# yskft04/NGT

Measured on AMD Instinct MI355X. Metric: QPS at recall@10=0.95, 1M x 128-d float L2; achieved HBM GB/s vs peak, higher is better.
Workload: dtype f32

## Files before the change

### include/ngt_amd.h

```cpp
#ifndef NGT_AMD_H
#define NGT_AMD_H

#include <stddef.h>
#include <stdint.h>

#ifdef __cplusplus
extern "C" {
#endif

#define NGT_AMD_DISTANCE_L1 0
#define NGT_AMD_DISTANCE_L2 1
#define NGT_AMD_DISTANCE_HAMMING 2
#define NGT_AMD_DISTANCE_ANGLE 3
#define NGT_AMD_DISTANCE_COSINE 4
#define NGT_AMD_DISTANCE_NORMALIZED_ANGLE 5
#define NGT_AMD_DISTANCE_NORMALIZED_COSINE 6
#define NGT_AMD_DISTANCE_JACCARD 7
#define NGT_AMD_DISTANCE_SPARSE_JACCARD 8
#define NGT_AMD_DISTANCE_NORMALIZED_L2 9
#define NGT_AMD_DISTANCE_POINCARE 100
#define NGT_AMD_DISTANCE_LORENTZ 101
#define NGT_AMD_OBJECT_UINT8 1
#define NGT_AMD_OBJECT_FLOAT 2

// ... 60 lines not shown

int ngt_amd_linear_search(ngt_amd_index *index, const void *queries, uint32_t nq, uint32_t k,
                          double radius, uint32_t *ids, float *dists, uint32_t *n);
int ngt_amd_linear_search_device(ngt_amd_index *index, const void *d_queries,
                                 uint64_t query_bytes, uint32_t nq, uint32_t k, double radius,
                                 uint32_t *d_ids, float *d_dists, uint32_t *d_n, void *stream);

int ngt_amd_distances(ngt_amd_index *index, const void *queries, uint32_t nq,
                      const uint32_t *qidx, const uint32_t *oid, uint64_t npairs, float *out);

int ngt_amd_prepare_queries_device(ngt_amd_index *index, const float *d_in, uint32_t nq,
                                   void *d_out, void *stream);

float ngt_amd_last_search_kernel_ms(const ngt_amd_index *index);
int ngt_amd_last_search_filtered(const ngt_amd_index *index);
int ngt_amd_stream_error_word(ngt_amd_index *index, void *stream, int *word);
uint32_t ngt_amd_last_search_slots(const ngt_amd_index *index);
uint32_t ngt_amd_last_search_budget(const ngt_amd_index *index);

#define NGT_AMD_GRAPH_ANNG 1
#define NGT_AMD_GRAPH_KNNG 2
#define NGT_AMD_GRAPH_ONNG 4
#define NGT_AMD_GRAPH_IANNG 5
typedef struct {
  int32_t edge_size_for_creation;
  int32_t edge_size_for_search;
  int32_t batch_size_for_creation;
  int32_t seed_size;
  float epsilon_for_creation;
  int32_t graph_type;
// ... 192 lines not shown
int ngt_amd_ngtq_open(const char *path, int device, ngt_amd_index **out);
int ngt_amd_ngtq_set(ngt_amd_index *index, const float *local, uint32_t N, uint32_t dsub,
                     const uint64_t *list_off, uint64_t nlists, const uint32_t *eids,
                     const uint16_t *elids, uint64_t nentries, const float *objects,
                     uint64_t object_records);
int ngt_amd_ngtq_search(ngt_amd_index *index, const ngt_amd_ngtq_search_params *params,
                        const float *queries, uint32_t nq, uint32_t *ids, float *dists, uint32_t *n);
int ngt_amd_ngtq_search_device(ngt_amd_index *index, const ngt_amd_ngtq_search_params *params,
                               const void *d_queries, uint64_t query_bytes, uint32_t nq,
                               uint32_t *d_ids, float *d_dists, uint32_t *d_n, void *stream);

int ngt_amd_test_unchecked_set(int device, int tagged, int trim, const uint64_t *script,
                               const uint8_t *tag_lane, uint32_t n, uint32_t tail_cap,
                               uint32_t spill_cap, float expr, uint64_t *popped, uint32_t *npopped,
                               uint64_t *events, uint32_t *nevents, uint32_t *maxq, uint32_t *error);

#ifdef __cplusplus
}
#endif
#endif
```

### ngt_amd/_sigs.py

```python
from ctypes import (POINTER, Structure, c_bool, c_char_p, c_double, c_float, c_int, c_int16, c_int32,
                    c_int64, c_size_t, c_uint, c_uint8, c_uint32, c_uint64, c_void_p)


class SearchParams(Structure):
    _fields_ = [("k", c_uint32), ("epsilon", c_float), ("radius", c_float), ("edge_size", c_int64),
                ("seed_mode", c_int32), ("all_leaf_nodes", c_int32),
                ("visited_hash_log2", c_int32), ("distance_filter", c_int32)]


class QgSearchParams(Structure):
    _fields_ = [("k", c_uint32), ("epsilon", c_float), ("result_expansion", c_float), ("radius", c_float),
                ("seed_mode", c_int32), ("visited_hash_log2", c_int32)]


class NgtqSearchParams(Structure):
    _fields_ = [("size", c_uint32), ("expansion", c_float), ("epsilon", c_float), ("mode", c_int32)]


class BuildParams(Structure):
    _fields_ = [("edge_size_for_creation", c_int32), ("edge_size_for_search", c_int32),
                ("batch_size_for_creation", c_int32), ("seed_size", c_int32), ("epsilon_for_creation", c_float),
                ("graph_type", c_int32)]


# ... 87 lines not shown
        "ngt_amd_last_search_lookahead": (c_int, [vp]),
        "ngt_amd_qg_train_local_ngt": (c_int, [vp, c_uint64, c_uint32, c_uint32, vp]),
        "ngt_amd_search_device": (c_int, [vp, POINTER(SearchParams), vp, c_uint64, c_uint32, vp, vp, vp, vp,
                                          vp, vp, vp]),
        "ngt_amd_linear_search": (c_int, [vp, vp, c_uint32, c_uint32, c_double, vp, vp, vp]),
        "ngt_amd_linear_search_device": (c_int, [vp, vp, c_uint64, c_uint32, c_uint32, c_double, vp, vp, vp,
                                                 vp]),
        "ngt_amd_distances": (c_int, [vp, vp, c_uint32, vp, vp, c_uint64, vp]),
        "ngt_amd_prepare_queries_device": (c_int, [vp, vp, c_uint32, vp, vp]),
        "ngt_amd_srand": (None, [c_uint]),
        "ngt_amd_last_search_kernel_ms": (c_float, [vp]),
        "ngt_amd_last_search_slots": (c_uint32, [vp]),
        "ngt_amd_stream_error_word": (c_int, [vp, vp, vp]),
        "ngt_amd_last_search_budget": (c_uint32, [vp]),
        "ngt_amd_last_search_filtered": (c_int, [vp]),
        "ngt_amd_build_begin": (c_int, [vp, POINTER(BuildParams)]),
        "ngt_amd_build_set_onng_edges": (c_int, [vp, c_int32, c_int32]),
        "ngt_amd_build_insert": (c_int, [vp, c_uint64, c_uint64]),
        "ngt_amd_build_graph_size": (c_int, [vp, u64p, u64p]),
        "ngt_amd_build_get_graph": (c_int, [vp, vp, vp, vp]),
        "ngt_amd_build_tree_size": (c_int, [vp, u32p, u32p, u64p]),
        "ngt_amd_build_get_tree": (c_int, [vp, vp, vp, vp, vp, vp, vp, vp, vp, vp, vp]),
        "ngt_amd_build_set_graph": (c_int, [vp, vp, vp, vp, c_uint64]),
        "ngt_amd_build_set_tree": (c_int, [vp, vp, vp, vp, vp, vp, vp, c_uint32, vp, vp, vp, vp, c_uint32,
                                           c_uint32]),
        "ngt_amd_build_remove": (c_int, [vp, vp, c_uint64, vp]),
        "ngt_amd_build_longest_removed_list": (c_uint64, [vp]),
        "ngt_amd_remove_relink": (c_int, [vp, vp, c_uint32, vp, vp, vp]),
        "ngt_amd_remove_fast_path_capacity": (c_uint32, []),
        "ngt_amd_onng_reconstruct": (c_int, [c_int, vp, vp, vp, c_uint64, POINTER(OnngParams), u64p]),
# ... 35 lines not shown
        "ngt_amd_qg_code_stride": (c_uint64, [vp]),
        "ngt_amd_qg_record_bytes": (c_uint64, [vp]),
        "ngt_amd_qg_get_graph": (c_int, [vp, vp, vp]),
        "ngt_amd_qg_lut": (c_int, [vp, vp, c_uint32, vp, vp, vp]),
        "ngt_amd_qg_adc": (c_int, [vp, vp, vp, vp, c_uint32, vp, vp, c_uint64, vp, vp]),
        "ngt_amd_qg_search": (c_int, [vp, POINTER(QgSearchParams), vp, c_uint32, vp, vp, vp, vp, vp, vp]),
        "ngt_amd_qg_search_device": (c_int, [vp, POINTER(QgSearchParams), vp, c_uint64, c_uint32, vp, vp, vp,
                                             vp, vp, vp, vp]),
        "ngt_amd_ngtq_open": (c_int, [c_char_p, c_int, POINTER(vp)]),
        "ngt_amd_ngtq_set": (c_int, [vp, vp, c_uint32, c_uint32, vp, c_uint64, vp, vp, c_uint64, vp, c_uint64]),
        "ngt_amd_ngtq_search": (c_int, [vp, POINTER(NgtqSearchParams), vp, c_uint32, vp, vp, vp]),
        "ngt_amd_ngtq_search_device": (c_int, [vp, POINTER(NgtqSearchParams), vp, c_uint64, c_uint32, vp, vp, vp,
                                               vp]),
        "ngt_amd_test_unchecked_set": (c_int, [c_int, c_int, c_int, vp, vp, c_uint32, c_uint32, c_uint32, c_float,
                                               vp, vp, vp, vp, vp, vp]),
        "ngt_open_index": (vp, [c_char_p, vp]),
        "ngt_create_graph_and_tree": (vp, [c_char_p, vp, vp]),
        "ngt_create_graph_and_tree_in_memory": (vp, [vp, vp]),
        "ngt_create_property": (vp, [vp]),
        "ngt_save_index": (c_bool, [vp, c_char_p, vp]),
        "ngt_get_property": (c_bool, [vp, vp, vp]),
        "ngt_get_property_dimension": (c_int32, [vp, vp]),
        "ngt_set_property_dimension": (c_bool, [vp, c_int32, vp]),
        "ngt_set_property_edge_size_for_creation": (c_bool, [vp, c_int16, vp]),
        "ngt_set_property_edge_size_for_search": (c_bool, [vp, c_int16, vp]),
        "ngt_get_property_object_type": (c_int32, [vp, vp]),
        "ngt_is_property_object_type_float": (c_bool, [c_int32]),
        "ngt_is_property_object_type_integer": (c_bool, [c_int32]),
        "ngt_set_property_object_type_float": (c_bool, [vp, vp]),
        "ngt_set_property_object_type_integer": (c_bool, [vp, vp]),
# ... 90 lines not shown
```

### ngt_amd/csrc/index_internal.h

```cpp
#pragma once
#include <hip/hip_runtime.h>
#include <stdint.h>

#include <algorithm>
#include <atomic>
#include <mutex>
#include <string>
#include <vector>

#include "../../include/ngt_amd.h"
#include "ngt_kernels.h"
#include "search_plan.h"

namespace ngt_amd {

int fail(const char* fmt, ...);

#define HIP_OK(expr)                                                                     \
  do {                                                                                   \
    hipError_t e_ = (expr);                                                              \
    if (e_ != hipSuccess)                                                                \
      return ngt_amd::fail("%s failed: %s (%s:%d)", #expr, hipGetErrorString(e_), __FILE__, __LINE__); \
  } while (0)

// ... 94 lines not shown
  DevBuf<float> local;
  DevBuf<uint64_t> list_off;
  DevBuf<uint32_t> eids;
  DevBuf<uint16_t> elids;
  DevBuf<uint8_t> orows;
};

struct SearchCtx {
  hipStream_t stream = nullptr;
  DevBuf<uint32_t> work, seeds, seed_count, slot_epoch;
  DevBuf<uint64_t> seed_off, spill;
  DevBuf<uint8_t> vis;
  uint32_t slots = 0;
  uint32_t launch_slots = 0;
  bool launch_filtered = false;
  int launch_la = -1;
  uint64_t vis_stride = 0;
  hipEvent_t ev0 = nullptr, ev1 = nullptr;
  DevBuf<uint8_t> lut;
  DevBuf<float> scale, toff;
  DevBuf<uint64_t> partial;
  DevBuf<uint16_t> sqh, sql;
  DevBuf<float> shb;
  DevBuf<uint64_t> gthr;
  DevBuf<uint32_t> ivf_cid, ivf_cn;
  DevBuf<float> ivf_cd;
  DevBuf<int> err;
  DevBuf<uint8_t> qstate;
  DevBuf<uint32_t> qflag, order;
  DevBuf<float> prio;
// ... 93 lines not shown
  uint64_t nrows = 0;
  DevBuf<uint8_t> rows, valid;
  uint64_t rows_version = 0;
  struct {
    DevBuf<uint16_t> rh, rl;
    DevBuf<uint32_t> xmax;
    uint64_t version = ~0ull;
    int passes = 0;
  } scan;
  struct {
    DevBuf<uint8_t> codes;
    DevBuf<uint32_t> st;
    DevBuf<float> params;
    uint64_t stride = 0;
    uint64_t version = ~0ull;
  } filt;
  std::vector<uint8_t> h_valid;
  std::vector<uint64_t> h_degree_nonzero;
  DevBuf<uint64_t> edge_off;
  DevBuf<uint32_t> edges;
  uint64_t nedges = 0;
  DevBuf<uint32_t> adj;
  uint64_t adj_stride = 0;
  uint64_t max_degree = 0;
  uint64_t adj_version = 0;

  bool has_graph = false;
  std::vector<uint8_t> h_graph_empty;
  bool has_tree = false;
  bool tree_has_empty_leaf = false;
// ... 81 lines not shown
```

### ngt_amd/csrc/ngt_amd_api.cpp

```cpp
#include <hip/hip_runtime.h>
#include <math.h>
#include <stdarg.h>
#include <stdio.h>
#include <stdlib.h>
#include <string.h>

#include <algorithm>
#include <climits>
#include <cmath>
#include <cfloat>
#include <string>
#include <vector>

#include "../../include/ngt_amd.h"
#include "device_graph.h"
#include "index_internal.h"
#include "ngt_kernels.h"
#include "prep_kernels.h"

using namespace ngt_amd;

static thread_local std::string g_err;

int ngt_amd::fail(const char* fmt, ...) {
// ... 372 lines not shown
  t.seed_stride = stride;
  t.seed_count = c->seed_count.p;
  HIP_OK(launch_tree_seeds(t, ix->metric, ix->otype, s));
  return 0;
}

static int ensure_filter(ngt_amd_index* ix) {
  std::lock_guard<std::mutex> lk(ix->mu);
  if (ix->filt.version == ix->rows_version) return 0;
  ix->filt.stride = ix->dp <= 128 ? ix->dp : (ix->dp + 127) / 128 * 128;
  HIP_OK(ix->filt.codes.alloc((size_t)ix->nrows * ix->filt.stride));
  HIP_OK(ix->filt.st.alloc(8));
  HIP_OK(ix->filt.params.alloc(8));
  HIP_OK(launch_filter_build(ix->rows.p, ix->row_bytes, ix->nrows, ix->dp, ix->filt.stride, ix->filt.codes.p, ix->filt.st.p,
                             ix->filt.params.p, ix->stream));
  HIP_OK(hipStreamSynchronize(ix->stream));
  ix->filt.version = ix->rows_version;
  return 0;
}

int ngt_amd::fill_index_args(ngt_amd_index* ix, uint64_t es, SearchArgs& a) {
  a.rows = ix->rows.p;
  a.row_bytes = ix->row_bytes;
  a.nrows = (uint32_t)ix->nrows;
  a.dp = (int)ix->dp;
  a.edge_off = ix->edge_off.p;
  a.edges = ix->edges.p;
  a.edge_size = es;
  std::lock_guard<std::mutex> lk(ix->mu);
  const uint64_t need = adjacency_need(ix, es);
  if (build_padded_adjacency(ix, need)) return -1;
// ... 146 lines not shown
  a.la_sh_log2 = plan.la_sh_log2;
  a.lat_slots = plan.lat_slots;
  a.lat_tail = plan.lat_tail;
  a.lat_hop = plan.lat_hop;
  a.lat_feed = plan.lat_feed;
  a.out_ids = d_ids;
  a.out_dists = d_dists;
  a.out_n = d_n;
  a.counters = d_counters;
  a.error = c->err.p;
  if (plan.use_filter) {
    if (ensure_filter(ix)) return -1;
    a.fcodes = ix->filt.codes.p;
    a.fstride = ix->filt.stride;
    a.fparams = ix->filt.params.p;
  }
  c->launch_filtered = plan.use_filter;

  if (prm->seed_mode == NGT_AMD_SEED_TREE) {
    if (run_tree_seeds(ix, c, d_queries, query_bytes, nq, prm->k, prm->all_leaf_nodes, s)) return -1;
    if (ix->tree_has_empty_leaf && !ix->h_graph_empty.empty() && fill_empty_tree_seeds(ix, c, nq, s)) return -1;
    a.seeds = c->seeds.p;
    a.seed_stride = kTreeSeedStride;
    a.seed_count = c->seed_count.p;
  } else {
    if (!d_seeds || !d_seed_off) return fail("search: seed lists required for this seed mode");
    a.seeds = d_seeds;
    a.seed_off = d_seed_off;
  }
  if (!plan.error.empty()) return fail("%s", plan.error.c_str());
  if (ensure_vis_scratch(ix, c, plan.lds_bytes, nq, s)) return -1;
  a.vis = c->vis.p;
  a.vis_stride = c->vis_stride;
  a.slot_epoch = c->slot_epoch.p;
  a.spill = c->spill.p;
  a.spill_cap = ix->spill_cap;
  a.work = c->work.p;
  HIP_OK(hipMemsetAsync(c->work.p, 0, 3 * sizeof(uint32_t), s));
  const uint32_t slots = std::min<uint32_t>(c->slots, nq);
  c->launch_slots = slots;
  c->launch_la = plan.la_mode();
  return launch_planned(ix, c, plan, a, slots, s);
}

static std::mutex g_rand_mu;
static GlibcRandHost& seed_rand() {
  static GlibcRandHost r = [] {
    GlibcRandHost g;
    g.seed(1);
    return g;
  }();
  return r;
}

extern "C" void ngt_amd_srand(unsigned int seed) {
// ... 97 lines not shown
  hipStream_t s = (hipStream_t)stream;
  SearchCtx* c = ctx_for(ix, s);
  if (!c) return -1;
  if (run_tree_seeds(ix, c, d_queries, query_bytes, nq, k, 0, s)) return -1;
  HIP_OK(hipMemcpy2DAsync(d_seeds, (size_t)seed_stride * sizeof(uint32_t), c->seeds.p,
                          (size_t)kTreeSeedStride * sizeof(uint32_t), (size_t)kTreeSeedStride * sizeof(uint32_t), nq,
                          hipMemcpyDeviceToDevice, s));
  HIP_OK(hipMemcpyAsync(d_count, c->seed_count.p, (size_t)nq * sizeof(uint32_t), hipMemcpyDeviceToDevice, s));
  return 0;
}

extern "C" int ngt_amd_last_search_filtered(const ngt_amd_index* ix) {
  if (!ix) return 0;
  SearchCtx* c = ix->last_ctx.load();
  return c && c->launch_filtered ? 1 : 0;
}

extern "C" int ngt_amd_last_search_lookahead(const ngt_amd_index* ix) {
  if (!ix) return -1;
  SearchCtx* c = ix->last_ctx.load();
  return c ? c->launch_la : -1;
}

extern "C" uint32_t ngt_amd_last_search_budget(const ngt_amd_index* ix) {
  if (!ix) return 0;
  SearchCtx* c = ix->last_ctx.load();
  return c ? c->launch_budget : 0;
}

extern "C" int ngt_amd_stream_error_word(ngt_amd_index* ix, void* stream, int* word) {
// ... 466 lines not shown
```

### ngt_amd/csrc/ngt_kernels.h

```cpp
#pragma once
#include <hip/hip_runtime.h>
#include <stddef.h>
#include <stdint.h>
#include <stdlib.h>

#include <algorithm>

#include "knobs.h"

namespace ngt_amd {

struct DistanceArgs {
  const uint8_t* rows;
  uint64_t row_bytes;
  const uint8_t* queries;
  uint64_t query_bytes;
  const uint32_t* qidx;
  const uint32_t* oid;
  float* out;
  uint64_t npairs;
  int dp;
};

struct TreeSeedArgs {
// ... 39 lines not shown
  const uint32_t* seeds;
  const uint64_t* seed_off;
  uint32_t seed_stride;
  const uint32_t* seed_count;
  uint32_t k;
  float coef;
  float radius;
  uint64_t edge_size;
  uint32_t ht_log2;
  uint32_t cq_cap;
  uint32_t vf_log2;
  uint32_t accepted_only;
  const uint8_t* fcodes;
  uint64_t fstride;
  const float* fparams;
  uint32_t* out_ids;
  float* out_dists;
  uint32_t* out_n;
  uint64_t* counters;
  uint32_t* work;
  uint8_t* vis;
  uint64_t vis_stride;
  uint32_t* slot_epoch;
  uint64_t* spill;
  uint32_t spill_cap;
  int* error;
  uint32_t la_lmax;
  uint32_t la_sh_log2;
  uint32_t lat_slots;
  uint32_t lat_tail;
// ... 407 lines not shown
```

### ngt_amd/csrc/search_common.h

```cpp
#pragma once
#include <hip/hip_runtime.h>
#include <stdint.h>

#include "ngt_device.h"

namespace ngt_amd {

#ifdef NGT_AMD_STAMPS
__device__ __forceinline__ uint64_t stamp() {
  uint64_t t;
  __builtin_amdgcn_sched_barrier(0);
  asm volatile("s_memtime %0\n\ts_waitcnt lgkmcnt(0)" : "=s"(t)::"memory");
  __builtin_amdgcn_sched_barrier(0);
  return t;
}
#define NGT_MARK(dst)              \
  do {                             \
    const uint64_t now_ = stamp(); \
    dst += now_ - t_last;          \
    t_last = now_;                 \
  } while (0)
#else
#define NGT_MARK(dst)
#endif
// ... 354 lines not shown
#pragma unroll
    for (int j = 0; j < 4; j++) {
      if (j == 0 || r0 + 16 * j < m) {
        uint32_t qc = 0u, cc = 0u;
#pragma unroll
        for (int w = 0; w < NW; w++) {
          qc = __builtin_amdgcn_udot4(q[w].x, c[j][w].x, qc, false);
          qc = __builtin_amdgcn_udot4(q[w].y, c[j][w].y, qc, false);
          cc = __builtin_amdgcn_udot4(c[j][w].x, c[j][w].x, cc, false);
          cc = __builtin_amdgcn_udot4(c[j][w].y, c[j][w].y, cc, false);
        }
        const uint32_t s = quad_sum_u32(cc - 2u * qc);
        const int r = r0 + 16 * j + rs;
        if (g == 0 && r < m) out[r] = sq + s;
      }
    }
  }
}

__device__ __forceinline__ void filter_query(const float* qf, int dp, float fa, float fb, uint8_t* qb, uint32_t& sq,
                                             double& rq) {
  uint32_t s = 0u;
  double r2 = 0.0;
  for (int i = lane_id(); i < dp; i += 64) {
    float c = rintf((qf[i] - fa) / fb);
    c = c >= 0.0f ? (c <= 255.0f ? c : 255.0f) : 0.0f;
    qb[i] = (uint8_t)c;
    s += (uint32_t)c * (uint32_t)c;
    double t = ((double)qf[i] - (double)fa) / (double)fb;
    t = t < 0.0 ? 0.0 : (t > 255.0 ? 255.0 : t);
// ... 124 lines not shown
```

### ngt_amd/csrc/search_kernels.hip

```cpp
#include <hip/hip_runtime.h>
#include <stdint.h>
#include <stdlib.h>

#include "ngt_device.h"
#include "ngt_kernels.h"
#include "search_common.h"
#include "search_layout.h"

namespace ngt_amd {



template <int M, typename T>
__global__ void __launch_bounds__(256) ngt_distances_kernel(DistanceArgs a) {
  const int lane = threadIdx.x & 63;
  const int g = lane & 3;
  const uint64_t quad = ((uint64_t)blockIdx.x * blockDim.x + threadIdx.x) >> 2;
  const uint64_t nquads = ((uint64_t)gridDim.x * blockDim.x) >> 2;
  for (uint64_t i = quad; i < a.npairs; i += nquads) {
    const T* q = reinterpret_cast<const T*>(a.queries + (uint64_t)a.qidx[i] * a.query_bytes);
    const T* x = row_ptr<T>(a.rows, a.row_bytes, a.oid[i]);
    const float d = quad_distance<M, T>(q, x, a.dp, g);
    if (g == 0) a.out[i] = d;
  }
// ... 128 lines not shown
    const uint64_t key = rsp[i];
    spill[i] = key;
    remark(key_id(key));
  }
  for (uint32_t i = lane; i < hv.npop; i += 64) remark(rpop[i]);
  __syncthreads();
}

#ifndef NGT_AMD_C2_WPE
#define NGT_AMD_C2_WPE 4
#endif
template <int M, int NCH, int G>
constexpr int search_waves_per_simd() {
  return (NCH > 0 && G == 1) ? NGT_AMD_C2_WPE : (NCH < 0 ? (M == kL2 ? 4 : 3) : 2);
}
template <int M, typename T, int NCH, int G>
__global__ void __launch_bounds__(64, (search_waves_per_simd<M, NCH, G>())) ngt_graph_search_kernel(SearchArgs a) {
  extern __shared__ __attribute__((aligned(16))) uint8_t smem[];
  const int lane = lane_id();
  SearchState st;
  uint8_t* p = smem;
  const bool use_hash = a.ht_log2 != 0;
  st.ht = reinterpret_cast<uint32_t*>(p);
  if (use_hash) p += (size_t)4 << a.ht_log2;
  st.vf = a.vf_log2 ? reinterpret_cast<uint32_t*>(p) : nullptr;
  st.vf_shift = 32 - a.vf_log2;
  const uint32_t vf_words = a.vf_log2 ? (1u << a.vf_log2) / 32 : 0u;
  p += (size_t)4 * vf_words;
  st.cq = reinterpret_cast<uint64_t*>(p);
  p += (size_t)8 * a.cq_cap;
  uint64_t* cmin = reinterpret_cast<uint64_t*>(p);
  p += ((size_t)8 * ((a.cq_cap + 63) / 64) + 15) & ~(size_t)15;
  st.res = reinterpret_cast<uint64_t*>(p);
  p += ((size_t)8 * (a.k + 1) + 15) & ~(size_t)15;
  st.nid = reinterpret_cast<uint32_t*>(p);
  p += 256;
  st.nd = reinterpret_cast<float*>(p);
  p += 256;
  T* qlds = reinterpret_cast<T*>(p);
  p += ((size_t)a.dp * sizeof(T) + 15) & ~(size_t)15;
  constexpr bool kFilterable = NCH > 0 && (NCH & 1) == 0 && M == kL2 && sizeof(T) == 4;
  constexpr bool kFilterCos = NCH < 0 && (M == kCosine || M == kAngle) && sizeof(T) == 4;
  uint8_t* qb = p;
  uint32_t* surv = reinterpret_cast<uint32_t*>(p + (size_t)a.dp);
  bool use_filter = false;
  float fa = 0.f, fb = 0.f, fe = 0.f, fx = 0.f;
  if constexpr (kFilterable || kFilterCos) {
    if (a.fcodes != nullptr && a.fparams[4] != 0.0f) {
      use_filter = true;
      fa = a.fparams[0];
      fb = a.fparams[1];
      fe = a.fparams[2];
      fx = a.fparams[3];
      use_filter = fb > 0.0f;
    }
  }
  (void)qb; (void)surv; (void)fa; (void)fb; (void)fe; (void)fx;

  const uint32_t slot = blockIdx.x;
  uint8_t* vis = a.vis + (uint64_t)slot * a.vis_stride;
  uint64_t* spill = a.spill + (uint64_t)slot * a.spill_cap;
  const uint32_t hcap = use_hash ? 1u << a.ht_log2 : 0u;
  const uint32_t hlimit = hcap - (hcap >> 2);

  const uint32_t nwork = a.nwork_dev ? *a.nwork_dev : a.nq;
  for (;;) {
    uint32_t w = 0;
    if (lane == 0) w = atomicAdd(a.work, 1u);
    w = (uint32_t)__builtin_amdgcn_readfirstlane((int)w);
// ... 23 lines not shown
        filter_query(reinterpret_cast<const float*>(qlds), a.dp, fa, fb, qb, fsq, frq);
        finv_b = 1.0 / (double)fb;
        __syncthreads();
      }
    }
    CosFilterQuery fcq{};
    (void)fcq;
    if constexpr (kFilterCos) {
      if (use_filter) {
        filter_query_cos(reinterpret_cast<const float*>(qlds), a.dp, fa, fb, qb, fcq);
        __syncthreads();
      }
    }

    bool bitmap_mode = !use_hash;
    const bool lazy = a.accepted_only && !use_hash && st.vf;
    uint32_t nvisited = 0;
    uint32_t ncq = 0, nspill = 0, nres = 0, maxq = 0;
    uint64_t ndist = 0, nvisit = 0, nexp = 0, nedge = 0, nexact = 0;
    uint64_t t_pop = 0, t_adj = 0, t_filt = 0, t_eval = 0, t_last = 0, t_rest = 0;
    (void)t_pop; (void)t_adj; (void)t_filt; (void)t_eval; (void)t_last; (void)t_rest;
#ifdef NGT_AMD_STAMPS
    t_last = stamp();
#endif
    float radius = a.radius;
    const uint32_t k = a.k;

    const uint64_t sb = a.seed_off ? a.seed_off[qi] : (uint64_t)qi * a.seed_stride;
    const uint32_t ns = a.seed_off ? (uint32_t)(a.seed_off[qi + 1] - sb) : a.seed_count[qi];
    if (resume) {
      PauseHdr h;
// ... 8 lines not shown
      nexp = h.nexp;
      nedge = h.nedge;
      nexact = h.nexact;
      for (uint32_t c = 0; c < ((ncq + 63) >> 6); c++) cq_chunk_min(st.cq, cmin, ncq, c);
      __syncthreads();
    }
    for (uint32_t base = 0; base < (resume ? 0u : ns); base += 64) {
      const uint32_t m = ns - base < 64 ? ns - base : 64;
      if ((uint32_t)lane < m) st.nid[lane] = a.seeds[sb + base + lane];
      __syncthreads();
      eval_any<M, T, NCH, G>(qlds, a, qfold, st.nid, st.nd, (int)m);
      __syncthreads();
      if ((uint32_t)lane < m) {
        const uint32_t id = st.nid[lane];
        const uint64_t key = make_key(st.nd[lane], id);
        visit(a.ht_log2, st, id, bitmap_mode, vis, epoch);
        if (ncq + lane < a.cq_cap) st.cq[ncq + lane] = key;
        else spill[nspill + (ncq + lane - a.cq_cap)] = key;
      }
      __syncthreads();
      for (uint32_t j = 0; j < m; j++) {
        const float d = st.nd[j];
        if (d <= a.radius) res_insert(st.res, nres, k, make_key(d, st.nid[j]));
      }
      const uint32_t ncq0 = ncq;
      if (ncq + m <= a.cq_cap) {
        ncq += m;
      } else {
        nspill += ncq + m - a.cq_cap;
        ncq = a.cq_cap;
      }
      for (uint32_t c = ncq0 >> 6; c < ((ncq + 63) >> 6); c++) cq_chunk_min(st.cq, cmin, ncq, c);
      ndist += m;
      nvisited += m;
      __syncthreads();
      if (!bitmap_mode && nvisited > hlimit) {
        ht_to_vis(a.ht_log2, st, vis, epoch);
        bitmap_mode = true;
        __syncthreads();
      }
    }
    if (nres >= k) radius = key_dist(st.res[k - 1]);
    float expr = __fmul_rn(a.coef, radius);

    auto accept_batch = [&](const uint32_t* ids, uint32_t me) {
      uint64_t okmask = ballot64((uint32_t)lane < me && st.nd[lane] <= expr);
      while (okmask) {
        const int j = __ffsll((long long)okmask) - 1;
        okmask &= okmask - 1;
        const float d = st.nd[j];
        if (!(d <= expr)) continue;
        const uint64_t key = make_key(d, ids[j]);
        if (lazy && lane == 0) mark_accepted(st, ids[j], vis, epoch);
        if (ncq >= a.cq_cap) {
          ncq = compact(st.cq, ncq, expr);
          if (nspill) nspill = compact(spill, nspill, expr);
          for (uint32_t c = 0; c < ((ncq + 63) >> 6); c++) cq_chunk_min(st.cq, cmin, ncq, c);
          __builtin_amdgcn_wave_barrier();
// ... 7 lines not shown
          ncq++;
        } else {
          if (nspill >= a.spill_cap) {
            if (lane == 0) atomicOr(a.error, 1);
          } else {
            if (lane == 0) spill[nspill] = key;
            nspill++;
          }
        }
        if (ncq + nspill > maxq) maxq = ncq + nspill;
        if (d <= radius) {
          res_insert(st.res, nres, k, key);
          if (nres >= k) {
            radius = key_dist(st.res[k - 1]);
            expr = __fmul_rn(a.coef, radius);
          }
        }
        __builtin_amdgcn_wave_barrier();
      }
      __syncthreads();
      if (!bitmap_mode && nvisited > hlimit) {
        ht_to_vis(a.ht_log2, st, vis, epoch);
        bitmap_mode = true;
        __syncthreads();
      }
    };

    uint32_t pf_node = 0, pf0 = 0, pf1 = 0, pf2 = 0, pf3 = 0;
    (void)pf_node; (void)pf0; (void)pf1; (void)pf2; (void)pf3;

// ... 42 lines not shown
      } else {
        ncq--;
        __syncthreads();
        cq_chunk_min(st.cq, cmin, ncq, bidx >> 6);
        if ((ncq >> 6) != (bidx >> 6)) cq_chunk_min(st.cq, cmin, ncq, ncq >> 6);
        __syncthreads();
      }
      nexp++;
      NGT_MARK(t_pop);

      const uint32_t target = key_id(wbest);
      if (a.pause_after && lane == 0 && nexp <= a.pause_after + kPauseStepMax)
        reinterpret_cast<uint32_t*>(a.qstate + (uint64_t)qi * a.qstate_stride +
                                    PauseLayout(a.k, a.cq_cap, 0).off_pop)[nexp - 1] = target;
      uint64_t eb, deg;
      const bool padded = a.adj != nullptr;
      if (padded) {
        eb = (uint64_t)target * a.adj_stride;
        deg = a.adj_stride < a.edge_size ? a.adj_stride : a.edge_size;
      } else {
        eb = a.edge_off[target];
        deg = a.edge_off[target + 1] - eb;
        if (deg > a.edge_size) deg = a.edge_size;
      }

      if constexpr (kFilterable) {
        if (use_filter && lazy && padded && deg <= 256) {
          const uint32_t nchk = (uint32_t)((deg + 63) >> 6);
          uint32_t a0, a1, a2, a3;
          if (pf_node == target) {
            a0 = pf0; a1 = pf1; a2 = pf2; a3 = pf3;
          } else {
            load_adj_row(a.adj + eb, deg, a0, a1, a2, a3);
          }
          {
            uint64_t nb = ~0ull;
            const uint32_t nc2 = (ncq + 63) >> 6;
            if ((uint32_t)lane < nc2) nb = cmin[lane];
            if ((uint32_t)lane + 64 < nc2) { const uint64_t v = cmin[lane + 64]; nb = v < nb ? v : nb; }
            for (uint32_t i = lane; i < nspill; i += 64) { const uint64_t v = spill[i]; nb = v < nb ? v : nb; }
            nb = wave_min_u64(nb);
            pf_node = (nb != ~0ull && key_dist(nb) <= expr) ? key_id(nb) : 0u;
// ... 4 lines not shown
          for (uint32_t c = 0; c < nchk; c++) {
            const uint32_t id = c == 0 ? a0 : (c == 1 ? a1 : (c == 2 ? a2 : a3));
            const uint64_t vmask = ballot64(id != 0u);
            const uint32_t cnt = (uint32_t)__popcll(vmask);
            nedge += cnt;
            if (cnt == 0) break;
            bool bit = false;
            uint32_t pw = 0;
            if (id != 0u) {
              const uint32_t b = (id * 0x85EBCA77u) >> st.vf_shift;
              bit = ((st.vf[b >> 5] >> (b & 31)) & 1u) != 0u;
              if (bit)
                pw = __hip_atomic_load(reinterpret_cast<const uint32_t*>(vis + (id & ~3u)), __ATOMIC_RELAXED,
                                       __HIP_MEMORY_SCOPE_AGENT);
            }
            st.nid[lane] = id;
            __syncthreads();
            filter_l2u8<NCH>(qb, fsq, a.fcodes, st.nid, reinterpret_cast<uint32_t*>(st.nd), (int)cnt);
            __syncthreads();
            const bool fresh = id != 0u && (!bit || ((pw >> (8 * (id & 3))) & 0xffu) != epoch);
            const uint32_t m = (uint32_t)__popcll(ballot64(fresh));
            ndist += m;
            nvisit += m;
            nvisited += m;
            const uint32_t fthr = filter_threshold(expr, (double)fe, finv_b, frq);
            const bool keep = fresh && reinterpret_cast<const uint32_t*>(st.nd)[lane] <= fthr;
            const uint64_t km = ballot64(keep);
            const uint32_t me = (uint32_t)__popcll(km);
            nexact += me;
            NGT_MARK(t_filt);
            if (ns + me > 64) {
              eval_any<M, T, NCH, G>(qlds, a, qfold, surv, st.nd, (int)ns);
              __syncthreads();
              NGT_MARK(t_eval);
              accept_batch(surv, ns);
              ns = 0;
            }
            if (keep) surv[ns + mbcnt(km)] = id;
            ns += me;
            __syncthreads();
// ... 365 lines not shown
}

hipError_t launch_schedule(const uint32_t* qflag, const float* prio, uint32_t nq, uint32_t* order, uint32_t* n_out,
                           hipStream_t s) {
  hipLaunchKernelGGL(ngt_schedule_kernel, dim3(1), dim3(1024), 0, s, qflag, prio, nq, order, n_out);
  return hipGetLastError();
}

hipError_t launch_graph_search(const SearchArgs& a, int metric, int otype, uint32_t slots,
                               hipStream_t s) {
  if (a.nq == 0) return hipSuccess;
  const size_t lds = search_lds_bytes(a, otype);
  if (metric == kL2 && otype == kFloat && (a.dp == 128 || a.dp == 96)) {
    if (a.dp == 128 && slots < 512)
      hipLaunchKernelGGL((ngt_graph_search_kernel<kL2, float, 8, 4>), dim3(slots), dim3(64), lds, s, a);
    else if (a.dp == 128)
      hipLaunchKernelGGL((ngt_graph_search_kernel<kL2, float, 8, 1>), dim3(slots), dim3(64), lds, s, a);
    else
      hipLaunchKernelGGL((ngt_graph_search_kernel<kL2, float, 6, 1>), dim3(slots), dim3(64), lds, s, a);
    return hipGetLastError();
  }
  if (otype == kFloat && a.dp > 128 && ((a.dp >> 4) & 3) == 0 && !ngt_amd::knob("NGT_AMD_NO_STREAM")) {
    if (metric == kL2) {
      hipLaunchKernelGGL((ngt_graph_search_kernel<kL2, float, -1, 1>), dim3(slots), dim3(64), lds, s, a);
      return hipGetLastError();
    }
    if (metric == kCosine) {
      hipLaunchKernelGGL((ngt_graph_search_kernel<kCosine, float, -1, 1>), dim3(slots), dim3(64), lds, s, a);
      return hipGetLastError();
    }
    if (metric == kAngle) {
      hipLaunchKernelGGL((ngt_graph_search_kernel<kAngle, float, -1, 1>), dim3(slots), dim3(64), lds, s, a);
// ... 61 lines not shown
```

### ngt_amd/csrc/search_plan.cpp

```cpp
#include "search_plan.h"

#include <stdio.h>
#include <stdlib.h>

#include <algorithm>

#include "knobs.h"
#include "search_layout.h"

namespace ngt_amd {

PlanKnobs read_plan_knobs() {
  PlanKnobs kn;
  kn.la = knob("NGT_AMD_LA");
  kn.filter = knob("NGT_AMD_FILTER");
  kn.no_stream = knob("NGT_AMD_NO_STREAM");
  kn.adj = knob("NGT_AMD_ADJ");
  kn.ht_log2 = knob("NGT_AMD_HT_LOG2");
  kn.cq_cap = knob("NGT_AMD_CQ_CAP");
  kn.accepted_only = knob("NGT_AMD_ACCEPTED_ONLY");
  kn.vfilter = knob("NGT_AMD_VFILTER");
  kn.la_lmax = knob("NGT_AMD_LA_LMAX");
  kn.lat = knob("NGT_AMD_LAT");
  kn.lat_tail = knob("NGT_AMD_LAT_TAIL");
  kn.lat_slots = knob("NGT_AMD_LAT_SLOTS");
  kn.lat_hop = knob("NGT_AMD_LAT_HOP");
  kn.lat_feed = knob("NGT_AMD_LAT_FEED");
  kn.sched = knob("NGT_AMD_SCHED");
  kn.sched_frac = knob("NGT_AMD_SCHED_FRAC");
  kn.sched_b = knob("NGT_AMD_SCHED_B");
  return kn;
}

void apply_visited_knobs(const PlanKnobs& kn, uint32_t& ht_log2, uint32_t& cq_cap, uint32_t& vf_log2,
                         bool keep_filter) {
  if (const char* v = kn.ht_log2) ht_log2 = (uint32_t)std::max(8, std::min(15, atoi(v)));
  if (const char* v = kn.cq_cap) cq_cap = (uint32_t)std::max(64, std::min(8192, atoi(v)));
  if (const char* v = kn.vfilter) {
    const int f = atoi(v);
    if (f > 0) vf_log2 = (uint32_t)std::max(11, std::min(18, f));
    else if (!keep_filter) vf_log2 = 0u;
  }
}

namespace {
// ... 141 lines not shown
  if (la_mode == 1 && !(kn.lat && atoi(kn.lat) == 0) && list_cap(sh) <= 256u && k <= 64u)
    lat = plan_speculating(sh, k, kn, p);
  if (!lat && la_mode >= 0 && la_lds(sh, k, p, la_mode) > lds_max) la_mode = -1;
  if (!lat) {
    p.kernel = la_mode < 0 ? kPlanOneExpansion : la_mode == 0 ? kPlanLookaheadWave : kPlanLookaheadEight;
    p.lds_bytes = la_mode >= 0 ? la_lds(sh, k, p, la_mode) : one_lds(sh, k, p);
  }
  p.la_full = la_mode >= 0 && !lat && !p.accepted_only;
  if (p.lds_bytes > lds_max) {
    char buf[160];
    snprintf(buf, sizeof buf, "search: k=%u needs %zu bytes of LDS per query (max %zu)", k, p.lds_bytes, lds_max);
    p.error = buf;
  }
  p.sched_shape = p.kernel == kPlanOneExpansion && p.accepted_only && p.ht_log2 == 0 && p.vf_log2 != 0 && p.use_adj &&
                  p.use_filter && k <= 64;
  p.sched_on = p.sched_shape && (kn.sched ? atoi(kn.sched) : 1) != 0;
  p.sched_frac = kn.sched_frac ? std::max(0.01, std::min(0.9, atof(kn.sched_frac))) : 0.25;
  p.sched_forced = kn.sched_b ? (uint32_t)std::max(0, atoi(kn.sched_b)) : 0u;
  return p;
}

}
```

### ngt_amd/csrc/search_plan.h

```cpp
#pragma once
#include <stddef.h>
#include <stdint.h>

#include <string>

#include "../../include/ngt_amd.h"

namespace ngt_amd {

struct PlanShape {
  int metric, otype;
  uint32_t dp;
  uint64_t row_bytes, nrows;
  int cu_count;
  size_t lds_per_block, lds_per_cu;
  uint64_t adj_stride;
  uint64_t edge_size;
};

struct PlanKnobs {
  const char *la, *filter, *no_stream, *adj, *ht_log2, *cq_cap, *accepted_only, *vfilter, *la_lmax, *lat, *lat_tail,
      *lat_slots, *lat_hop, *lat_feed, *sched, *sched_frac, *sched_b;
};
PlanKnobs read_plan_knobs();

enum PlanKernel : int {
  kPlanOneExpansion = 0,
  kPlanLookaheadWave,
  kPlanLookaheadEight,
  kPlanSpeculating,
};

struct SearchPlan {
  PlanKernel kernel = kPlanOneExpansion;
  uint32_t ht_log2 = 12, cq_cap = 1024, vf_log2 = 0, accepted_only = 0;
  bool use_adj = false;
  bool use_filter = false;
  uint32_t la_lmax = 0, la_sh_log2 = 0;
  bool la_full = false;
  uint32_t lat_slots = 0, lat_tail = 0, lat_hop = 0, lat_feed = 0;
  size_t lds_bytes = 0;
  bool sched_shape = false;
  bool sched_on = false;
  double sched_frac = 0.25;
  uint32_t sched_forced = 0;
  std::string error;
  int la_mode() const { return kernel == kPlanOneExpansion ? -1 : kernel == kPlanLookaheadWave ? 0 : 1; }
};

SearchPlan plan_search(const PlanShape& sh, const ngt_amd_search_params& prm, uint32_t nq, const PlanKnobs& kn);

bool plan_speculating(const PlanShape& sh, uint32_t k, const PlanKnobs& kn, SearchPlan& p);

void apply_visited_knobs(const PlanKnobs& kn, uint32_t& ht_log2, uint32_t& cq_cap, uint32_t& vf_log2,
                         bool keep_filter = false);

}
// ... 1 lines not shown
```

### ngt_amd/device.py

```python
import ctypes
from ctypes import byref, c_void_p

import numpy as np

from . import NativeError, lib
from ._sigs import QgSearchParams, SearchParams

DISTANCE = {
    "l1": 0, "l2": 1, "hamming": 2, "angle": 3, "cosine": 4, "normalized_angle": 5,
    "normalized_cosine": 6, "jaccard": 7, "sparse_jaccard": 8, "normalized_l2": 9,
    "poincare": 100, "lorentz": 101,
}
SEED_TREE, SEED_GIVEN, SEED_RANDOM = 0, 1, 2
COUNTERS = 8
GRAPH_ANNG, GRAPH_KNNG, GRAPH_ONNG, GRAPH_IANNG = 1, 2, 4, 5


def padded_dim(dim):
    return ((dim - 1) // 16 + 1) * 16


def _chk(rc):
    if rc != 0:
        raise NativeError(lib().ngt_amd_last_error().decode())
# ... 151 lines not shown
        return s.value, l.value

    def search_device(self, d_queries, query_bytes, nq, d_ids, d_dists, d_n, d_counters=None, k=10,
                      epsilon=0.1, radius=-1.0, edge_size=-1, seed_mode=SEED_TREE, d_seeds=None,
                      d_seed_off=None, stream=None, visited_hash_log2=0, distance_filter=0):
        prm = SearchParams(k, epsilon, radius, edge_size, seed_mode, 0, visited_hash_log2, distance_filter)
        _chk(self.L.ngt_amd_search_device(self.h, byref(prm), d_queries, query_bytes, nq, d_seeds, d_seed_off,
                                          d_ids, d_dists, d_n, d_counters, stream))

    def last_search_kernel_ms(self):
        return float(self.L.ngt_amd_last_search_kernel_ms(self.h))

    def last_search_filtered(self):
        return bool(self.L.ngt_amd_last_search_filtered(self.h))

    def last_search_lookahead(self):
        return int(self.L.ngt_amd_last_search_lookahead(self.h))

    def last_search_budget(self):
        return int(self.L.ngt_amd_last_search_budget(self.h))

    def last_search_slots(self):
        return int(self.L.ngt_amd_last_search_slots(self.h))

    def prepare_queries_device(self, d_in, nq, d_out, stream=None):
        _chk(self.L.ngt_amd_prepare_queries_device(self.h, d_in, nq, d_out, stream))

    def linear_search(self, queries, k=10, radius=-1.0):
        q = np.ascontiguousarray(queries, dtype=np.float32)
        nq = q.shape[0]
# ... 197 lines not shown
```

Before: 741,200.

## Add specialized production variant of filtered L2 float graph search kernel

```diff
diff --git a/include/ngt_amd.h b/include/ngt_amd.h
--- a/include/ngt_amd.h
+++ b/include/ngt_amd.h
@@ -98,6 +98,7 @@
 
 float ngt_amd_last_search_kernel_ms(const ngt_amd_index *index);
 int ngt_amd_last_search_filtered(const ngt_amd_index *index);
+int ngt_amd_last_search_production(const ngt_amd_index *index);
 int ngt_amd_stream_error_word(ngt_amd_index *index, void *stream, int *word);
 uint32_t ngt_amd_last_search_slots(const ngt_amd_index *index);
 uint32_t ngt_amd_last_search_budget(const ngt_amd_index *index);
@@ -320,6 +321,9 @@
                                const uint8_t *tag_lane, uint32_t n, uint32_t tail_cap,
                                uint32_t spill_cap, float expr, uint64_t *popped, uint32_t *npopped,
                                uint64_t *events, uint32_t *nevents, uint32_t *maxq, uint32_t *error);
+int ngt_amd_test_filter_chunk(int device, const uint8_t *codes, uint32_t nrows, uint32_t dp,
+                              const uint8_t *qb, const uint32_t *ids, const uint32_t *cnt,
+                              uint32_t ncase, uint32_t *out);
 
 #ifdef __cplusplus
 }
diff --git a/ngt_amd/_sigs.py b/ngt_amd/_sigs.py
--- a/ngt_amd/_sigs.py
+++ b/ngt_amd/_sigs.py
@@ -125,6 +125,7 @@
         "ngt_amd_stream_error_word": (c_int, [vp, vp, vp]),
         "ngt_amd_last_search_budget": (c_uint32, [vp]),
         "ngt_amd_last_search_filtered": (c_int, [vp]),
+        "ngt_amd_last_search_production": (c_int, [vp]),
         "ngt_amd_build_begin": (c_int, [vp, POINTER(BuildParams)]),
         "ngt_amd_build_set_onng_edges": (c_int, [vp, c_int32, c_int32]),
         "ngt_amd_build_insert": (c_int, [vp, c_uint64, c_uint64]),
@@ -190,6 +191,7 @@
                                                vp]),
         "ngt_amd_test_unchecked_set": (c_int, [c_int, c_int, c_int, vp, vp, c_uint32, c_uint32, c_uint32, c_float,
                                                vp, vp, vp, vp, vp, vp]),
+        "ngt_amd_test_filter_chunk": (c_int, [c_int, vp, c_uint32, c_uint32, vp, vp, vp, c_uint32, vp]),
         "ngt_open_index": (vp, [c_char_p, vp]),
         "ngt_create_graph_and_tree": (vp, [c_char_p, vp, vp]),
         "ngt_create_graph_and_tree_in_memory": (vp, [vp, vp]),
diff --git a/ngt_amd/csrc/index_internal.h b/ngt_amd/csrc/index_internal.h
--- a/ngt_amd/csrc/index_internal.h
+++ b/ngt_amd/csrc/index_internal.h
@@ -132,6 +132,7 @@
   uint32_t slots = 0;
   uint32_t launch_slots = 0;
   bool launch_filtered = false;
+  bool launch_production = false;
   int launch_la = -1;
   uint64_t vis_stride = 0;
   hipEvent_t ev0 = nullptr, ev1 = nullptr;
@@ -255,6 +256,7 @@
     DevBuf<float> params;
     uint64_t stride = 0;
     uint64_t version = ~0ull;
+    bool usable = false;
   } filt;
   std::vector<uint8_t> h_valid;
   std::vector<uint64_t> h_degree_nonzero;
diff --git a/ngt_amd/csrc/ngt_amd_api.cpp b/ngt_amd/csrc/ngt_amd_api.cpp
--- a/ngt_amd/csrc/ngt_amd_api.cpp
+++ b/ngt_amd/csrc/ngt_amd_api.cpp
@@ -410,7 +410,10 @@
   HIP_OK(ix->filt.params.alloc(8));
   HIP_OK(launch_filter_build(ix->rows.p, ix->row_bytes, ix->nrows, ix->dp, ix->filt.stride, ix->filt.codes.p, ix->filt.st.p,
                              ix->filt.params.p, ix->stream));
+  float h_params[5];
+  HIP_OK(hipMemcpyAsync(h_params, ix->filt.params.p, sizeof h_params, hipMemcpyDeviceToHost, ix->stream));
   HIP_OK(hipStreamSynchronize(ix->stream));
+  ix->filt.usable = h_params[4] != 0.0f && h_params[1] > 0.0f;
   ix->filt.version = ix->rows_version;
   return 0;
 }
@@ -587,6 +590,7 @@
     a.fcodes = ix->filt.codes.p;
     a.fstride = ix->filt.stride;
     a.fparams = ix->filt.params.p;
+    a.production = plan.production && ix->filt.usable;
   }
   c->launch_filtered = plan.use_filter;
 
@@ -612,6 +616,8 @@
   HIP_OK(hipMemsetAsync(c->work.p, 0, 3 * sizeof(uint32_t), s));
   const uint32_t slots = std::min<uint32_t>(c->slots, nq);
   c->launch_slots = slots;
+  if (a.dp == 128 && slots < 512) a.production = 0;
+  c->launch_production = a.production != 0;
   c->launch_la = plan.la_mode();
   return launch_planned(ix, c, plan, a, slots, s);
 }
@@ -739,6 +745,12 @@
   if (!ix) return 0;
   SearchCtx* c = ix->last_ctx.load();
   return c && c->launch_filtered ? 1 : 0;
+}
+
+extern "C" int ngt_amd_last_search_production(const ngt_amd_index* ix) {
+  if (!ix) return 0;
+  SearchCtx* c = ix->last_ctx.load();
+  return c && c->launch_production ? 1 : 0;
 }
 
 extern "C" int ngt_amd_last_search_lookahead(const ngt_amd_index* ix) {
diff --git a/ngt_amd/csrc/ngt_kernels.h b/ngt_amd/csrc/ngt_kernels.h
--- a/ngt_amd/csrc/ngt_kernels.h
+++ b/ngt_amd/csrc/ngt_kernels.h
@@ -77,6 +77,7 @@
   const uint8_t* fcodes;
   uint64_t fstride;
   const float* fparams;
+  uint32_t production;
   uint32_t* out_ids;
   float* out_dists;
   uint32_t* out_n;
diff --git a/ngt_amd/csrc/search_common.h b/ngt_amd/csrc/search_common.h
--- a/ngt_amd/csrc/search_common.h
+++ b/ngt_amd/csrc/search_common.h
@@ -392,6 +392,43 @@
         const int r = r0 + 16 * j + rs;
         if (g == 0 && r < m) out[r] = sq + s;
       }
+    }
+  }
+}
+
+template <int NCH>
+__device__ __forceinline__ void filter_l2u8_chunk(const uint8_t* qb, uint32_t sq, const uint8_t* codes, uint32_t id,
+                                                  uint32_t* out, uint32_t cnt) {
+  static_assert((NCH & 1) == 0, "whole 8-byte code words per lane");
+  constexpr int E = 4 * NCH;
+  constexpr int NW = E / 8;
+  const int lane = lane_id();
+  const int g = lane & 3, rs = lane >> 2;
+  uint32_t rid[4];
+#pragma unroll
+  for (int j = 0; j < 4; j++) rid[j] = (uint32_t)__builtin_amdgcn_ds_bpermute(4 * (16 * j + rs), (int)id);
+  uint2 c[4][NW];
+#pragma unroll
+  for (int j = 0; j < 4; j++) {
+    if (j == 0 || 16u * j < cnt) load_code_words<NW>(codes + (uint64_t)rid[j] * (4 * E) + g * (8 * NW), c[j]);
+  }
+  uint2 q[NW];
+  const uint2* qp = reinterpret_cast<const uint2*>(qb + g * E);
+#pragma unroll
+  for (int w = 0; w < NW; w++) q[w] = qp[w];
+#pragma unroll
+  for (int j = 0; j < 4; j++) {
+    if (j == 0 || 16u * j < cnt) {
+      uint32_t qc = 0u, cc = 0u;
+#pragma unroll
+      for (int w = 0; w < NW; w++) {
+        qc = __builtin_amdgcn_udot4(q[w].x, c[j][w].x, qc, false);
+        qc = __builtin_amdgcn_udot4(q[w].y, c[j][w].y, qc, false);
+        cc = __builtin_amdgcn_udot4(c[j][w].x, c[j][w].x, cc, false);
+        cc = __builtin_amdgcn_udot4(c[j][w].y, c[j][w].y, cc, false);
+      }
+      const uint32_t s = quad_sum_u32(cc - 2u * qc);
+      if (g == 0) out[16 * j + rs] = sq + s;
     }
   }
 }
diff --git a/ngt_amd/csrc/search_kernels.hip b/ngt_amd/csrc/search_kernels.hip
--- a/ngt_amd/csrc/search_kernels.hip
+++ b/ngt_amd/csrc/search_kernels.hip
@@ -166,13 +166,15 @@
 constexpr int search_waves_per_simd() {
   return (NCH > 0 && G == 1) ? NGT_AMD_C2_WPE : (NCH < 0 ? (M == kL2 ? 4 : 3) : 2);
 }
-template <int M, typename T, int NCH, int G>
+template <int M, typename T, int NCH, int G, bool PROD = false>
 __global__ void __launch_bounds__(64, (search_waves_per_simd<M, NCH, G>())) ngt_graph_search_kernel(SearchArgs a) {
+  static_assert(!PROD || (NCH > 0 && (NCH & 1) == 0 && M == kL2 && sizeof(T) == 4 && G == 1),
+                "the production variant is the filtered L2 float form");
   extern __shared__ __attribute__((aligned(16))) uint8_t smem[];
   const int lane = lane_id();
   SearchState st;
   uint8_t* p = smem;
-  const bool use_hash = a.ht_log2 != 0;
+  const bool use_hash = !PROD && a.ht_log2 != 0;
   st.ht = reinterpret_cast<uint32_t*>(p);
   if (use_hash) p += (size_t)4 << a.ht_log2;
   st.vf = a.vf_log2 ? reinterpret_cast<uint32_t*>(p) : nullptr;
@@ -198,13 +200,13 @@
   bool use_filter = false;
   float fa = 0.f, fb = 0.f, fe = 0.f, fx = 0.f;
   if constexpr (kFilterable || kFilterCos) {
-    if (a.fcodes != nullptr && a.fparams[4] != 0.0f) {
+    if (PROD || (a.fcodes != nullptr && a.fparams[4] != 0.0f)) {
       use_filter = true;
       fa = a.fparams[0];
       fb = a.fparams[1];
       fe = a.fparams[2];
       fx = a.fparams[3];
-      use_filter = fb > 0.0f;
+      use_filter = PROD || fb > 0.0f;
     }
   }
   (void)qb; (void)surv; (void)fa; (void)fb; (void)fe; (void)fx;
@@ -258,7 +260,7 @@
     }
 
     bool bitmap_mode = !use_hash;
-    const bool lazy = a.accepted_only && !use_hash && st.vf;
+    const bool lazy = PROD || (a.accepted_only && !use_hash && st.vf);
     uint32_t nvisited = 0;
     uint32_t ncq = 0, nspill = 0, nres = 0, maxq = 0;
     uint64_t ndist = 0, nvisit = 0, nexp = 0, nedge = 0, nexact = 0;
@@ -297,7 +299,7 @@
       if ((uint32_t)lane < m) {
         const uint32_t id = st.nid[lane];
         const uint64_t key = make_key(st.nd[lane], id);
-        visit(a.ht_log2, st, id, bitmap_mode, vis, epoch);
+        visit(PROD ? 0u : a.ht_log2, st, id, bitmap_mode, vis, epoch);
         if (ncq + lane < a.cq_cap) st.cq[ncq + lane] = key;
         else spill[nspill + (ncq + lane - a.cq_cap)] = key;
       }
@@ -325,6 +327,9 @@
     }
     if (nres >= k) radius = key_dist(st.res[k - 1]);
     float expr = __fmul_rn(a.coef, radius);
+    uint32_t fthr_q = 0u;
+    (void)fthr_q;
+    if constexpr (PROD) fthr_q = filter_threshold(expr, (double)fe, finv_b, frq);
 
     auto accept_batch = [&](const uint32_t* ids, uint32_t me) {
       uint64_t okmask = ballot64((uint32_t)lane < me && st.nd[lane] <= expr);
@@ -362,6 +367,7 @@
           if (nres >= k) {
             radius = key_dist(st.res[k - 1]);
             expr = __fmul_rn(a.coef, radius);
+            if constexpr (PROD) fthr_q = filter_threshold(expr, (double)fe, finv_b, frq);
           }
         }
         __builtin_amdgcn_wave_barrier();
@@ -434,7 +440,7 @@
         reinterpret_cast<uint32_t*>(a.qstate + (uint64_t)qi * a.qstate_stride +
                                     PauseLayout(a.k, a.cq_cap, 0).off_pop)[nexp - 1] = target;
       uint64_t eb, deg;
-      const bool padded = a.adj != nullptr;
+      const bool padded = PROD || a.adj != nullptr;
       if (padded) {
         eb = (uint64_t)target * a.adj_stride;
         deg = a.adj_stride < a.edge_size ? a.adj_stride : a.edge_size;
@@ -445,7 +451,7 @@
       }
 
       if constexpr (kFilterable) {
-        if (use_filter && lazy && padded && deg <= 256) {
+        if (PROD || (use_filter && lazy && padded && deg <= 256)) {
           const uint32_t nchk = (uint32_t)((deg + 63) >> 6);
           uint32_t a0, a1, a2, a3;
           if (pf_node == target) {
@@ -480,16 +486,20 @@
                 pw = __hip_atomic_load(reinterpret_cast<const uint32_t*>(vis + (id & ~3u)), __ATOMIC_RELAXED,
                                        __HIP_MEMORY_SCOPE_AGENT);
             }
-            st.nid[lane] = id;
-            __syncthreads();
-            filter_l2u8<NCH>(qb, fsq, a.fcodes, st.nid, reinterpret_cast<uint32_t*>(st.nd), (int)cnt);
+            if constexpr (PROD) {
+              filter_l2u8_chunk<NCH>(qb, fsq, a.fcodes, id, reinterpret_cast<uint32_t*>(st.nd), cnt);
+            } else {
+              st.nid[lane] = id;
+              __syncthreads();
+              filter_l2u8<NCH>(qb, fsq, a.fcodes, st.nid, reinterpret_cast<uint32_t*>(st.nd), (int)cnt);
+            }
             __syncthreads();
             const bool fresh = id != 0u && (!bit || ((pw >> (8 * (id & 3))) & 0xffu) != epoch);
             const uint32_t m = (uint32_t)__popcll(ballot64(fresh));
             ndist += m;
             nvisit += m;
             nvisited += m;
-            const uint32_t fthr = filter_threshold(expr, (double)fe, finv_b, frq);
+            const uint32_t fthr = PROD ? fthr_q : filter_threshold(expr, (double)fe, finv_b, frq);
             const bool keep = fresh && reinterpret_cast<const uint32_t*>(st.nd)[lane] <= fthr;
             const uint64_t km = ballot64(keep);
             const uint32_t me = (uint32_t)__popcll(km);
@@ -885,8 +895,12 @@
   if (metric == kL2 && otype == kFloat && (a.dp == 128 || a.dp == 96)) {
     if (a.dp == 128 && slots < 512)
       hipLaunchKernelGGL((ngt_graph_search_kernel<kL2, float, 8, 4>), dim3(slots), dim3(64), lds, s, a);
+    else if (a.dp == 128 && a.production)
+      hipLaunchKernelGGL((ngt_graph_search_kernel<kL2, float, 8, 1, true>), dim3(slots), dim3(64), lds, s, a);
     else if (a.dp == 128)
       hipLaunchKernelGGL((ngt_graph_search_kernel<kL2, float, 8, 1>), dim3(slots), dim3(64), lds, s, a);
+    else if (a.production)
+      hipLaunchKernelGGL((ngt_graph_search_kernel<kL2, float, 6, 1, true>), dim3(slots), dim3(64), lds, s, a);
     else
       hipLaunchKernelGGL((ngt_graph_search_kernel<kL2, float, 6, 1>), dim3(slots), dim3(64), lds, s, a);
     return hipGetLastError();
diff --git a/ngt_amd/csrc/search_plan.cpp b/ngt_amd/csrc/search_plan.cpp
--- a/ngt_amd/csrc/search_plan.cpp
+++ b/ngt_amd/csrc/search_plan.cpp
@@ -29,6 +29,7 @@
   kn.sched = knob("NGT_AMD_SCHED");
   kn.sched_frac = knob("NGT_AMD_SCHED_FRAC");
   kn.sched_b = knob("NGT_AMD_SCHED_B");
+  kn.prod = knob("NGT_AMD_PROD");
   return kn;
 }
 
@@ -200,6 +201,9 @@
   }
   p.sched_shape = p.kernel == kPlanOneExpansion && p.accepted_only && p.ht_log2 == 0 && p.vf_log2 != 0 && p.use_adj &&
                   p.use_filter && k <= 64;
+  p.production = p.sched_shape && sh.metric == NGT_AMD_DISTANCE_L2 && sh.otype == NGT_AMD_OBJECT_FLOAT &&
+                 (sh.dp == 128 || sh.dp == 96) && list_cap(sh) <= 256 &&
+                 !(kn.prod && atoi(kn.prod) == 0);
   p.sched_on = p.sched_shape && (kn.sched ? atoi(kn.sched) : 1) != 0;
   p.sched_frac = kn.sched_frac ? std::max(0.01, std::min(0.9, atof(kn.sched_frac))) : 0.25;
   p.sched_forced = kn.sched_b ? (uint32_t)std::max(0, atoi(kn.sched_b)) : 0u;
diff --git a/ngt_amd/csrc/search_plan.h b/ngt_amd/csrc/search_plan.h
--- a/ngt_amd/csrc/search_plan.h
+++ b/ngt_amd/csrc/search_plan.h
@@ -20,7 +20,7 @@
 
 struct PlanKnobs {
   const char *la, *filter, *no_stream, *adj, *ht_log2, *cq_cap, *accepted_only, *vfilter, *la_lmax, *lat, *lat_tail,
-      *lat_slots, *lat_hop, *lat_feed, *sched, *sched_frac, *sched_b;
+      *lat_slots, *lat_hop, *lat_feed, *sched, *sched_frac, *sched_b, *prod;
 };
 PlanKnobs read_plan_knobs();
 
@@ -41,6 +41,7 @@
   uint32_t lat_slots = 0, lat_tail = 0, lat_hop = 0, lat_feed = 0;
   size_t lds_bytes = 0;
   bool sched_shape = false;
+  bool production = false;
   bool sched_on = false;
   double sched_frac = 0.25;
   uint32_t sched_forced = 0;
diff --git a/ngt_amd/device.py b/ngt_amd/device.py
--- a/ngt_amd/device.py
+++ b/ngt_amd/device.py
@@ -189,6 +189,9 @@
     def last_search_filtered(self):
         return bool(self.L.ngt_amd_last_search_filtered(self.h))
 
+    def last_search_production(self):
+        return bool(self.L.ngt_amd_last_search_production(self.h))
+
     def last_search_lookahead(self):
         return int(self.L.ngt_amd_last_search_lookahead(self.h))
 
```

Result: no change. 741,700, median of 4 (+0.1%).
